# automl/TransformersCanDoBayesianInference

Hardware: AMD Instinct MI355X
Metric: synthetic datasets/sec (GP prior, bptt=2000) (higher is better)
Workload: dtype fp16; 1 GPU; priors.fast_gp, bptt=2000, num_features=18, emsize=512, nhead=4, nhid=1024, nlayers=6, 1000 bars (BASELINE.json configs[1]); per_gpu_batch=64, global_batch=64, aggregate_k_gradients=1, aggregate_streams=0, aggregate_stacked=False, seq_len=2000, parallelism=dp1, micro_batch_streams=2, eval_pos=weighted sampler(2000)

## Files before the change

transformerscandobayesianinference_amd/csrc/gemm.hip:

```cpp
#include <type_traits>
#include "pfn_device.h"
#include "pfn_kernels.h"

namespace pfn {

PFN_DEV int xcd_remap(int bid, int nwg) {
  const int q = nwg >> 3, r = nwg & 7, xcd = bid & 7;
  return (xcd < r ? xcd * (q + 1) : r * (q + 1) + (xcd - r) * q) + (bid >> 3);
}

constexpr int GEMM_BM = 128, GEMM_BN = 128, GEMM_RB = 128;

template <typename T>
__global__ __launch_bounds__(256, 2) void gemm_nt_kernel(GemmNT g) {
  operand_store_mode<T>();
  constexpr int BK = GEMM_RB / sizeof(T);
  extern __shared__ __attribute__((aligned(16))) char smem_raw[];
  LdsPtr smem = lds_cast(smem_raw);
  auto tileA = [&](int buf) { return smem + buf * 32768; };
  auto tileB = [&](int buf) { return smem + buf * 32768 + 16384; };

  const int tiles_n = (g.N + GEMM_BN - 1) / GEMM_BN;
  const int tiles_m = (g.M + GEMM_BM - 1) / GEMM_BM;
  const int tid_lin = xcd_remap(blockIdx.x, tiles_m * tiles_n);
  const int tm = tid_lin / tiles_n, tn = tid_lin % tiles_n;
  const int m0 = tm * GEMM_BM, n0 = tn * GEMM_BN;
  const int rowsA = min(GEMM_BM, g.M - m0), rowsB = min(GEMM_BN, g.N - n0);

  const T* A = reinterpret_cast<const T*>(g.A) + (long)m0 * g.lda;
  const T* B = reinterpret_cast<const T*>(g.B) + (long)n0 * g.ldb;

  const int wave = threadIdx.x >> 6, lane = threadIdx.x & 63;
  const int wm = wave >> 1, wn = wave & 1;

  f32x16 acc[2][2];
#pragma unroll
  for (int i = 0; i < 2; ++i)
#pragma unroll
    for (int j = 0; j < 2; ++j)
#pragma unroll
      for (int r = 0; r < 16; ++r) acc[i][j][r] = 0.f;

  TileStage<T, GEMM_BM, GEMM_RB, 256> sa, sb;
  const int nk = (g.K + BK - 1) / BK;
  sa.issue(A, g.lda, rowsA, g.K);
  sb.issue(B, g.ldb, rowsB, g.K);
  sa.template commit<false>(tileA(0));
  sb.template commit<false>(tileB(0));
  __syncthreads();

  for (int kt = 0; kt < nk; ++kt) {
    const int cur = kt & 1;
    if (kt + 1 < nk) {
      const int k1 = (kt + 1) * BK;
      sa.issue(A + k1, g.lda, rowsA, g.K - k1);
      sb.issue(B + k1, g.ldb, rowsB, g.K - k1);
    }
    const lds_char* ta = tileA(cur);
    const lds_char* tb = tileB(cur);
#pragma unroll
    for (int ks = 0; ks < BK; ks += 16) {
// ... 78 lines not shown
        const int n = ncol + e;
        if (flags & EPI_BIAS) x += bias[n];
        if ((flags & EPI_ROWSHIFT) && n >= g.rs_n0 && n < g.rs_n1) x -= g.rowshift[(m / g.rs_S) * g.rs_ld + (n - g.rs_n0)];
        if (flags & EPI_GELU_BWD) x *= (float)aux[m * g.ld_aux + n];
        if (flags & EPI_RESID) x += g.resid[m * g.ld_resid + n];
        if (flags & EPI_RESID_T) x += (float)aux[m * g.ld_aux + n];
        float second = x;
        if (flags & EPI_GELU) gelu_and_grad(x, x, second);
        if (flags & EPI_OUT2_T) out2_t[m * g.ld_out2 + n] = (T)second;
        if (flags & EPI_OUT_F32) { float* o = g.out_f32 + m * g.ld_out_f32 + n; *o = (flags & EPI_ACCUM) ? (*o + x) : x; }
        if (flags & EPI_OUT_T) out_t[m * g.ld_out_t + n] = (T)x;
      }
    }
  }
}


constexpr int BIG_BN = 256;
template <int NWM> struct BigEpi {
  static constexpr int EP_T = 32 * 144, EP_F = 32 * 272, EP_WAVE = (2 * EP_T > EP_F ? 2 * EP_T : EP_F), BYTES = NWM * 4 * EP_WAVE;
};
template <typename T, int FLAGS, int NWM>
PFN_DEV void nt_big_epilogue(const GemmNT& g, f32x16 (&acc)[4][2], int m0, int n0, int wave, int lane, LdsPtr ep_base, const lds_char* shift_lds = nullptr) {
  const int wm = wave >> 2, wn = wave & 3;
  const int h = lane >> 5, li = lane & 31;
  constexpr int flags = FLAGS;
  const T* aux = reinterpret_cast<const T*>(g.aux);
  T* out_t = reinterpret_cast<T*>(g.out_t);
  T* out2_t = reinterpret_cast<T*>(g.out2_t);
  constexpr bool HAS_AUX = (flags & (EPI_GELU_BWD | EPI_RESID_T | EPI_ROWDOT)) != 0;
  constexpr bool HAS_RES = (flags & EPI_RESID) != 0;
  float rowdot = 0.f;
  constexpr bool EARLY = NWM == 2;
  constexpr int NB = !EARLY ? 1 : HAS_RES ? 2 : 4;
  f32x4 bias_v[2][4];
  if ((flags & EPI_BIAS) && EARLY) {
#pragma unroll
    for (int j = 0; j < 2; ++j)
#pragma unroll
      for (int gq = 0; gq < 4; ++gq) bias_v[j][gq] = *reinterpret_cast<const f32x4*>(g.bias + min(n0 + wn * 64 + j * 32 + 8 * gq + 4 * h, g.N - 4));
  }
  constexpr int EP_T = 32 * 144, EP_F = 32 * 272, EP_WAVE = (2 * EP_T > EP_F ? 2 * EP_T : EP_F);
  static_assert(!(flags & EPI_ACCUM), "accumulating outputs take the generic kernel");
  LdsPtr ep = ep_base + wave * EP_WAVE;
  const bool lines = n0 + wn * 64 + 64 <= g.N && g.wide_t;
#pragma unroll
  for (int pass = 0; pass < 8 / NB; ++pass) {
    X4<T> aux_v[HAS_AUX ? NB : 1][4];
    f32x4 res_v[HAS_RES ? NB : 1][4];
#pragma unroll
    for (int bb = 0; bb < NB; ++bb) {
      const int blk = pass * NB + bb, i = blk >> 1, j = blk & 1;
      if (EARLY && (HAS_AUX || HAS_RES)) {
        const long m = min((long)m0 + wm * 128 + i * 32 + li, (long)g.M - 1);
#pragma unroll
        for (int gq = 0; gq < 4; ++gq) {
          const int n = min(n0 + wn * 64 + j * 32 + 8 * gq + 4 * h, g.N - 4);
          if constexpr (HAS_AUX) aux_v[bb][gq] = *reinterpret_cast<const X4<T>*>(aux + m * g.ld_aux + n);
          if constexpr (HAS_RES) res_v[bb][gq] = *reinterpret_cast<const f32x4*>(g.resid + m * g.ld_resid + n);
        }
      }
    }
#pragma unroll
    for (int bb = 0; bb < NB; ++bb) {
      const int blk = pass * NB + bb, i = blk >> 1, j = blk & 1;
      const long m_row = (long)m0 + wm * 128 + i * 32 + li;
      const bool mvalid = m_row < g.M;
      const long m = mvalid ? m_row : (long)g.M - 1;
      const int nb = n0 + wn * 64 + j * 32;
      float pre[16], post[16];
      f32x4 shift_v[4];
      const bool shifted = (flags & EPI_ROWSHIFT) && nb >= g.rs_n0 && nb < g.rs_n1;
      if (shifted) {
        if (shift_lds) {
          const int which = min((int)((unsigned)m / (unsigned)g.rs_S) - (int)((unsigned)m0 / (unsigned)g.rs_S), 1);
          const lds_char* sp = shift_lds + (which * BIG_BN + (nb - n0) + 4 * h) * 4;
#pragma unroll
          for (int gq = 0; gq < 4; ++gq) shift_v[gq] = __builtin_bit_cast(f32x4, lds_read16(sp + 32 * gq));
        } else {
          const float* sp = g.rowshift + (long)((unsigned)m / (unsigned)g.rs_S) * g.rs_ld + (nb - g.rs_n0) + 4 * h;
#pragma unroll
          for (int gq = 0; gq < 4; ++gq) shift_v[gq] = *reinterpret_cast<const f32x4*>(sp + 8 * gq);
        }
      }
#pragma unroll
      for (int gq = 0; gq < 4; ++gq) {
        const int n = min(nb + 8 * gq + 4 * h, g.N - 4);
        f32x4 v;
#pragma unroll
        for (int e = 0; e < 4; ++e) v[e] = acc[i][j][4 * gq + e];
        if constexpr (!EARLY) {
          if (flags & EPI_BIAS) bias_v[j][gq] = *reinterpret_cast<const f32x4*>(g.bias + n);
          if constexpr (HAS_AUX) aux_v[bb][gq] = *reinterpret_cast<const X4<T>*>(aux + m * g.ld_aux + n);
          if constexpr (HAS_RES) res_v[bb][gq] = *reinterpret_cast<const f32x4*>(g.resid + m * g.ld_resid + n);
        }
        if (flags & EPI_BIAS) v += bias_v[j][gq];
        if (shifted) v -= shift_v[gq];
        if (flags & EPI_GELU_BWD) {
#pragma unroll
          for (int e = 0; e < 4; ++e) v[e] *= (float)aux_v[HAS_AUX ? bb : 0][gq][e];
        }
        if (flags & EPI_RESID) v += res_v[HAS_RES ? bb : 0][gq];
        if (flags & EPI_RESID_T) {
#pragma unroll
          for (int e = 0; e < 4; ++e) v[e] += (float)aux_v[HAS_AUX ? bb : 0][gq][e];
        }
#pragma unroll
// ... 199 lines not shown

template <int NWN> struct LnEpi {
  static constexpr int STRIPS = 128 * NWN * 4 + 5 * NWN * 64 * 4;
  static constexpr int WAVE = 32 * 272 + 32 * 144;
  static constexpr int BYTES = STRIPS + NWN * WAVE;
};
template <typename T, int NWN, bool RESID_LN, int BK, bool Y16>
__global__ __launch_bounds__(NWN * 64) void gemm_nt_ln_kernel(GemmLN g) {
  operand_store_mode<T>();
  constexpr int BM = 128, RB = BK * 2, CPR = RB / 16, RPP = 1024 / RB, BN = NWN * 64;
  constexpr int PA = BM / RPP / NWN > 0 ? BM / RPP / NWN : 1, PB = BN / RPP / NWN;
  constexpr int TILE_A = BM * RB, STAGE = TILE_A + BN * RB;
  extern __shared__ __attribute__((aligned(16))) char smem_raw[];
  LdsPtr smem = lds_cast(smem_raw);
  const int m0 = blockIdx.x * BM;
  const int wave = __builtin_amdgcn_readfirstlane(threadIdx.x >> 6), lane = threadIdx.x & 63;
  const int h = lane >> 5, li = lane & 31;

  const T* pa[PA];
  const T* pb[PB];
  constexpr int APIECES = BM / RPP;
#pragma unroll
  for (int i = 0; i < PA; ++i) {
    const int piece = wave + NWN * i;
    const int row = piece * RPP + lane / CPR;
    const int chunk = swz16<RB>(row, lane % CPR);
    pa[i] = reinterpret_cast<const T*>(g.A) + (long)min(m0 + row, g.M - 1) * g.lda + chunk * 8;
  }
#pragma unroll
  for (int i = 0; i < PB; ++i) {
    const int row = (wave + NWN * i) * RPP + lane / CPR;
    const int chunk = swz16<RB>(row, lane % CPR);
    pb[i] = reinterpret_cast<const T*>(g.B) + (long)row * g.ldb + chunk * 8;
  }
  auto stage = [&](int buf, int k0) {
    LdsPtr ta = smem + buf * STAGE + wave * 1024;
    LdsPtr tb = smem + buf * STAGE + TILE_A + wave * 1024;
#pragma unroll
    for (int i = 0; i < PA; ++i)
      if (wave + NWN * i < APIECES) __builtin_amdgcn_global_load_lds((gvoid_t*)(pa[i] + k0), (lvoid_t*)(ta + i * NWN * 1024), 16, 0, 0);
#pragma unroll
    for (int i = 0; i < PB; ++i) __builtin_amdgcn_global_load_lds((gvoid_t*)(pb[i] + k0), (lvoid_t*)(tb + i * NWN * 1024), 16, 0, 0);
  };

  f32x16 acc[4][2];
#pragma unroll
  for (int i = 0; i < 4; ++i)
#pragma unroll
    for (int j = 0; j < 2; ++j)
#pragma unroll
      for (int r = 0; r < 16; ++r) acc[i][j][r] = 0.f;

  const int nk = g.K / BK;
  stage(0, 0);
  __syncthreads();
  for (int kt = 0; kt < nk; ++kt) {
    const int cur = kt & 1;
    if (kt + 1 < nk) stage(cur ^ 1, (kt + 1) * BK);
    const lds_char* ta = smem + cur * STAGE;
    const lds_char* tb = ta + TILE_A;
#pragma unroll
    for (int ks = 0; ks < BK; ks += 16) {
      Frag<T> fa[4], fb[2];
#pragma unroll
      for (int j = 0; j < 2; ++j) fb[j] = load_frag_row<T, RB>(tb, wave * 64 + j * 32 + li, ks);
#pragma unroll
      for (int i = 0; i < 4; ++i) fa[i] = load_frag_row<T, RB>(ta, i * 32 + li, ks);
#pragma unroll
      for (int i = 0; i < 4; ++i)
#pragma unroll
        for (int j = 0; j < 2; ++j) acc[i][j] = mma32(fb[j], fa[i], acc[i][j]);
    }
    __syncthreads();
  }

  float* red = reinterpret_cast<float*>(smem_raw);
  float* cvec = red + 128 * NWN;
  {
    const int n = threadIdx.x;
    float c0 = 0.f, c1 = 0.f;
    if constexpr (RESID_LN) { c0 = g.rgamma[n]; c1 = g.rbeta[n]; }
    const float c2 = g.bias[n], c3 = g.gamma[n], c4 = g.beta[n];
    cvec[n] = c0; cvec[BN + n] = c1; cvec[2 * BN + n] = c2; cvec[3 * BN + n] = c3; cvec[4 * BN + n] = c4;
  }
  typedef typename std::conditional<Y16 && RESID_LN, X4<T>, f32x4>::type RV;
  const float* rsrc = RESID_LN ? reinterpret_cast<const float*>(g.ry) : g.resid;
  float rm[2], rr[2];
  int mrow[4];
#pragma unroll
  for (int i = 0; i < 4; ++i) mrow[i] = min(m0 + i * 32 + li, g.M - 1);
  RV rv[2][8];
  auto fetch_rows = [&](int i, RV (&dst)[8]) {
    rm[i & 1] = 0.f; rr[i & 1] = 1.f;
    if constexpr (RESID_LN) { rm[i & 1] = g.rmean[mrow[i]]; rr[i & 1] = g.rrstd[mrow[i]]; }
#pragma unroll
    for (int j = 0; j < 2; ++j)
#pragma unroll
      for (int gq = 0; gq < 4; ++gq) {
        const long off = (long)mrow[i] * BN + wave * 64 + j * 32 + 8 * gq + 4 * h;
        if constexpr (Y16 && RESID_LN) dst[j * 4 + gq] = *reinterpret_cast<const X4<T>*>(reinterpret_cast<const T*>(g.ry) + off);
        else dst[j * 4 + gq] = *reinterpret_cast<const f32x4*>(rsrc + off);
      }
  };
  fetch_rows(0, rv[0]);
  __syncthreads();
  float mean[4], rstd[4];
  const float invN = 1.f / (float)BN;
#pragma unroll
  for (int i = 0; i < 4; ++i) {
    if (i + 1 < 4) fetch_rows(i + 1, rv[(i + 1) & 1]);
    float s = 0.f;
#pragma unroll
    for (int j = 0; j < 2; ++j)
#pragma unroll
      for (int gq = 0; gq < 4; ++gq) {
        const int n = wave * 64 + j * 32 + 8 * gq + 4 * h;
        f32x4 r;
#pragma unroll
        for (int e = 0; e < 4; ++e) r[e] = (float)rv[i & 1][j * 4 + gq][e];
        if constexpr (RESID_LN) {
          const f32x4 ga = *reinterpret_cast<const f32x4*>(cvec + n), be = *reinterpret_cast<const f32x4*>(cvec + BN + n);
#pragma unroll
          for (int e = 0; e < 4; ++e) r[e] = (r[e] - rm[i & 1]) * rr[i & 1] * ga[e] + be[e];
        }
        const f32x4 bi = *reinterpret_cast<const f32x4*>(cvec + 2 * BN + n);
#pragma unroll
        for (int e = 0; e < 4; ++e) {
          const float v = acc[i][j][4 * gq + e] + bi[e] + r[e];
          acc[i][j][4 * gq + e] = v;
          s += v;
        }
      }
    s += __shfl_xor(s, 32, 64);
    if (h == 0) red[(i * 32 + li) * NWN + wave] = s;
  }
  __syncthreads();
#pragma unroll
  for (int i = 0; i < 4; ++i) {
    float t = 0.f;
#pragma unroll
    for (int w = 0; w < NWN; ++w) t += red[(i * 32 + li) * NWN + w];
    mean[i] = t * invN;
  }
  __syncthreads();
#pragma unroll
  for (int i = 0; i < 4; ++i) {
    float s = 0.f;
#pragma unroll
    for (int j = 0; j < 2; ++j)
#pragma unroll
      for (int r = 0; r < 16; ++r) { const float d = acc[i][j][r] - mean[i]; s += d * d; }
    s += __shfl_xor(s, 32, 64);
    if (h == 0) red[(i * 32 + li) * NWN + wave] = s;
  }
  __syncthreads();
#pragma unroll
  for (int i = 0; i < 4; ++i) {
    float t = 0.f;
#pragma unroll
    for (int w = 0; w < NWN; ++w) t += red[(i * 32 + li) * NWN + w];
    rstd[i] = rsqrtf(t * invN + g.eps);
  }
  typedef __attribute__((address_space(3))) X4<T> lds_tx4;
  T* x_t = reinterpret_cast<T*>(g.x_t);
  LdsPtr sf = smem + LnEpi<NWN>::STRIPS + wave * LnEpi<NWN>::WAVE, st = sf + 32 * 272;
#pragma unroll
  for (int i = 0; i < 4; ++i) {
    const bool mvalid = m0 + i * 32 + li < g.M;
    const long m = mrow[i];
    if (mvalid && wave == 0 && h == 0) { g.mean[m] = mean[i]; g.rstd[m] = rstd[i]; }
#pragma unroll
    for (int j = 0; j < 2; ++j) {
      const int nb = wave * 64 + j * 32;
#pragma unroll
      for (int gq = 0; gq < 4; ++gq) {
        const int n = nb + 8 * gq + 4 * h;
        const f32x4 ga = *reinterpret_cast<const f32x4*>(cvec + 3 * BN + n), be = *reinterpret_cast<const f32x4*>(cvec + 4 * BN + n);
        f32x4 v, xo;
        X4<T> xt;
#pragma unroll
        for (int e = 0; e < 4; ++e) {
          v[e] = acc[i][j][4 * gq + e];
          xo[e] = (v[e] - mean[i]) * rstd[i] * ga[e] + be[e];
          xt[e] = (T)xo[e];
        }
        if constexpr (Y16) {
          X4<T> vt;
// ... 328 lines not shown
  for (int i = 0; i < 4; ++i)
#pragma unroll
    for (int j = 0; j < 2; ++j)
#pragma unroll
      for (int r = 0; r < 16; ++r) acc[i][j][r] = 0.f;

  const int nk = g.K / BK;
  stage(0, 0);
  __syncthreads();
  for (int kt = 0; kt < nk; ++kt) {
    const int cur = kt & 1;
    if (kt + 1 < nk) stage(cur ^ 1, (kt + 1) * BK);
    const lds_char* ta = smem + cur * STAGE;
    const lds_char* tb = ta + TILE_A;
#pragma unroll
    for (int ks = 0; ks < BK; ks += 16) {
      Frag<T> fa[4], fb[2];
#pragma unroll
      for (int j = 0; j < 2; ++j) fb[j] = load_frag_row<T, RB>(tb, wave * 64 + j * 32 + li, ks);
#pragma unroll
      for (int i = 0; i < 4; ++i) fa[i] = load_frag_row<T, RB>(ta, i * 32 + li, ks);
#pragma unroll
      for (int i = 0; i < 4; ++i)
#pragma unroll
        for (int j = 0; j < 2; ++j) acc[i][j] = mma32(fb[j], fa[i], acc[i][j]);
    }
    __syncthreads();
  }

  typedef __attribute__((address_space(3))) X4<T> lds_tx4;
  float* red1 = reinterpret_cast<float*>(smem_raw);
  float* red2 = red1 + 128 * NWN;
  float* gam = red2 + 128 * NWN;
  LdsPtr stash = smem + C::STASH + wave * 4 * C::STRIP;
  const T* aux = reinterpret_cast<const T*>(g.aux);
  T* dx_t = reinterpret_cast<T*>(g.dx_t);
  gam[threadIdx.x] = g.gamma[threadIdx.x];
  int mrow[4];
  bool mvalid[4];
  float mu[4], rs[4];
#pragma unroll
  for (int i = 0; i < 4; ++i) {
    const int m = m0 + i * 32 + li;
    mvalid[i] = m < g.M;
    mrow[i] = mvalid[i] ? m : g.M - 1;
    mu[i] = g.mean[mrow[i]]; rs[i] = g.rstd[mrow[i]];
  }
  typedef typename std::conditional<Y16, X4<T>, f32x4>::type YV;
  YV yv[2][4];
  X4<T> av[2][4];
  auto fetch_half = [&](int hb, YV (&dy)[4], X4<T> (&da)[4]) {
#pragma unroll
    for (int gq = 0; gq < 4; ++gq) {
      const long off = (long)mrow[hb >> 1] * BN + wave * 64 + (hb & 1) * 32 + 8 * gq + 4 * h;
      if constexpr (Y16) dy[gq] = *reinterpret_cast<const X4<T>*>(reinterpret_cast<const T*>(g.y) + off);
      else dy[gq] = *reinterpret_cast<const f32x4*>(reinterpret_cast<const float*>(g.y) + off);
      da[gq] = *reinterpret_cast<const X4<T>*>(aux + off);
    }
  };
  fetch_half(0, yv[0], av[0]);
  __syncthreads();
  const float invN = 1.f / (float)BN;
  float s1 = 0.f, s2 = 0.f;
#pragma unroll
  for (int hb = 0; hb < 8; ++hb) {
    const int i = hb >> 1, j = hb & 1;
    asm volatile("" ::: "memory");
    if (hb + 1 < 8) fetch_half(hb + 1, yv[(hb + 1) & 1], av[(hb + 1) & 1]);
    __builtin_amdgcn_sched_barrier(0);
#pragma unroll
    for (int gq = 0; gq < 4; ++gq) {
      const int n = wave * 64 + j * 32 + 8 * gq + 4 * h;
      const f32x4 ga = *reinterpret_cast<const f32x4*>(gam + n);
      X4<T> xh_t;
#pragma unroll
      for (int e = 0; e < 4; ++e) {
        const float v = mvalid[i] ? acc[i][j][4 * gq + e] + (float)av[hb & 1][gq][e] : 0.f;
        acc[i][j][4 * gq + e] = v;
        const float xh = ((float)yv[hb & 1][gq][e] - mu[i]) * rs[i];
        const float gv = ga[e] * v;
        s1 += gv;
        s2 += gv * xh;
        xh_t[e] = (T)xh;
      }
      *reinterpret_cast<lds_tx4*>(stash + i * C::STRIP + li * 144 + (j * 4 + gq) * 16 + h * 8) = xh_t;
    }
    if (j == 1) {
      s1 += __shfl_xor(s1, 32, 64);
      s2 += __shfl_xor(s2, 32, 64);
      if (h == 0) { red1[(i * 32 + li) * NWN + wave] = s1; red2[(i * 32 + li) * NWN + wave] = s2; }
      s1 = 0.f; s2 = 0.f;
    }
  }
  __syncthreads();
  float m1[4], m2[4];
#pragma unroll
  for (int i = 0; i < 4; ++i) {
    float t1 = 0.f, t2 = 0.f;
#pragma unroll
    for (int w = 0; w < NWN; ++w) { t1 += red1[(i * 32 + li) * NWN + w]; t2 += red2[(i * 32 + li) * NWN + w]; }
    m1[i] = t1 * invN; m2[i] = t2 * invN;
  }
  __syncthreads();
  float* csum = red1;
  const int ccol = wave * 64 + 4 * h, chalf = (li >> 4) * BN;
  {
#pragma unroll
// ... 338 lines not shown
    PFN_BIG_CASE(EPI_OUT_T | EPI_ROWDOT)
    PFN_BIG_CASE(EPI_OUT_F32)
    PFN_BIG_CASE(EPI_BIAS | EPI_OUT_F32)
#undef PFN_BIG_CASE
    default: return false;
  }
}

static void nt_prepare(GemmNT& g, int precision);
bool gemm_nt_rowdot_fused(const GemmNT& g_in, int precision) {
  GemmNT g = g_in;
  if (!prec_is16(precision) || g.M <= 0 || g.flags != (EPI_OUT_T | EPI_ROWDOT) || g.N % 64 || g.rd_D % 64 || g.N % g.rd_D) return false;
  if ((g.lda * 2) % 16 || (g.ldb * 2) % 16 || !aligned16(g.A) || !aligned16(g.B)) return false;
  nt_prepare(g, precision);
  return gemm_nt_pick(g) == 1 && g.wide_t;
}
int launch_gemm_nt(const GemmNT& g_in, int precision, hipStream_t stream) {
  GemmNT g = g_in;
  if (g.M <= 0 || g.N <= 0 || g.K <= 0) return PFN_OK;
  const size_t es = prec_esize(precision);
  if ((g.lda * es) % 16 || (g.ldb * es) % 16 || !aligned16(g.A) || !aligned16(g.B)) return PFN_ERR_ALIGNMENT;
  if ((g.flags & EPI_ROWSHIFT) && (!g.rowshift || g.rs_S <= 0 || g.rs_n0 % 64 || g.rs_n1 % 64 || g.rs_n0 < 0 || g.rs_n1 > g.N)) return PFN_ERR_ARGUMENT;
  nt_prepare(g, precision);
  if (prec_is16(precision)) {
    const int pick = gemm_nt_pick(g);
    if (pick && (precision == PFN_PREC_FP16 ? launch_big<f16>(g, pick == 2, stream) : launch_big<bf16>(g, pick == 2, stream)))
      return hipGetLastError() == hipSuccess ? PFN_OK : PFN_ERR_LAUNCH;
  }
  if (g.flags & EPI_ROWDOT) return PFN_ERR_UNSUPPORTED;
  const int tiles = ((g.M + GEMM_BM - 1) / GEMM_BM) * ((g.N + GEMM_BN - 1) / GEMM_BN);
  PFN_DISPATCH_OP(precision, hipLaunchKernelGGL(gemm_nt_kernel<T>, dim3(tiles), dim3(256), 65536, stream, g));
  return hipGetLastError() == hipSuccess ? PFN_OK : PFN_ERR_LAUNCH;
}
static void nt_prepare(GemmNT& g, int precision) {
  const size_t es = prec_esize(precision);
  bool vec = true;
  if ((g.flags & EPI_OUT_F32) && (g.ld_out_f32 % 4 || !aligned16(g.out_f32))) vec = false;
  if ((g.flags & EPI_OUT_T) && ((g.ld_out_t * es) % (4 * es) || !aligned16(g.out_t))) vec = false;
  if ((g.flags & EPI_OUT2_T) && ((g.ld_out2 * es) % (4 * es) || !aligned16(g.out2_t))) vec = false;
  if ((g.flags & EPI_RESID) && (g.ld_resid % 4 || !aligned16(g.resid))) vec = false;
  if ((g.flags & (EPI_GELU_BWD | EPI_RESID_T | EPI_ROWDOT)) && ((g.ld_aux * es) % (4 * es) || !aligned16(g.aux))) vec = false;
  if ((g.flags & EPI_BIAS) && !aligned16(g.bias)) vec = false;
  if ((g.flags & EPI_ROWSHIFT) && (!aligned16(g.rowshift) || g.rs_ld % 4 || g.rs_n0 % 4 || g.rs_n1 % 4)) vec = false;
  g.vec_ok = vec ? 1 : 0;
  g.wide_t = (!(g.flags & EPI_OUT_T) || g.ld_out_t % 8 == 0) && (!(g.flags & EPI_OUT2_T) || g.ld_out2 % 8 == 0) ? 1 : 0;
}

bool gemm_ln_supported(const GemmLN& g) {
  return (g.N == 128 || g.N == 256 || g.N == 512 || g.N == 1024) && g.K % 32 == 0 && g.K >= 32 && (g.lda * 2) % 16 == 0 && (g.ldb * 2) % 16 == 0 &&
         aligned16(g.A) && aligned16(g.B) && aligned16(g.bias) && aligned16(g.gamma) && aligned16(g.beta) && aligned16(g.y) && aligned16(g.x_t) &&
         (g.resid ? aligned16(g.resid) : (aligned16(g.ry) && aligned16(g.rgamma) && aligned16(g.rbeta)));
}
template <typename T, bool Y, int NWN, bool RL, int BK> static void launch_gemm_ln_t(const GemmLN& g, hipStream_t stream) {
  const size_t lds = std::max<size_t>(2 * (128 + NWN * 64) * (BK * 2), LnEpi<NWN>::BYTES);
  static LdsAllowance allowance;
  allowance.ensure(gemm_nt_ln_kernel<T, NWN, RL, BK, Y>, lds);
  hipLaunchKernelGGL((gemm_nt_ln_kernel<T, NWN, RL, BK, Y>), dim3((g.M + 127) / 128), dim3(NWN * 64), lds, stream, g);
}
static int g_ln_rows64 = 0;
void set_gemm_ln_rows64(int on) { g_ln_rows64 = on; }
template <typename T, bool Y, int NWN, bool RL, int BK, int MI, int NJ> static void launch_gemm_ln_wide_t(const GemmLN& g, hipStream_t stream) {
  constexpr int BM = MI * 32;
  const size_t lds = std::max<size_t>(2 * (BM + NWN * NJ * 32) * (BK * 2), LnEpiW<NWN, MI, NJ>::BYTES);
  static LdsAllowance allowance;
  allowance.ensure(gemm_nt_ln_wide_kernel<T, NWN, RL, BK, MI, NJ, Y>, lds);
  hipLaunchKernelGGL((gemm_nt_ln_wide_kernel<T, NWN, RL, BK, MI, NJ, Y>), dim3((g.M + BM - 1) / BM), dim3(NWN * 64), lds, stream, g);
}
template <typename T, bool Y> static int launch_gemm_ln_op(const GemmLN& g, hipStream_t stream) {
  const bool rl = g.resid == nullptr;
#define PFN_LN_CASE(NWN) \
  if (g.K % 64 == 0) { if (rl) launch_gemm_ln_t<T, Y, NWN, true, 64>(g, stream); else launch_gemm_ln_t<T, Y, NWN, false, 64>(g, stream); } \
  else { if (rl) launch_gemm_ln_t<T, Y, NWN, true, 32>(g, stream); else launch_gemm_ln_t<T, Y, NWN, false, 32>(g, stream); }
  if (g.N == 512 && g_ln_rows64) {
    if (rl) launch_gemm_ln_wide_t<T, Y, 4, true, 32, 2, 4>(g, stream); else launch_gemm_ln_wide_t<T, Y, 4, false, 32, 2, 4>(g, stream);
    return hipGetLastError() == hipSuccess ? PFN_OK : PFN_ERR_LAUNCH;
  }
  switch (g.N / 64) {
    case 2: PFN_LN_CASE(2) break;
    case 4: PFN_LN_CASE(4) break;
    case 8: PFN_LN_CASE(8) break;
    default:
      if (rl) launch_gemm_ln_wide_t<T, Y, 8, true, 32, 2, 4>(g, stream); else launch_gemm_ln_wide_t<T, Y, 8, false, 32, 2, 4>(g, stream);
      break;
  }
#undef PFN_LN_CASE
  return hipGetLastError() == hipSuccess ? PFN_OK : PFN_ERR_LAUNCH;
}
int launch_gemm_ln(const GemmLN& g, int precision, hipStream_t stream) {
  if (g.M <= 0) return PFN_OK;
  if (!prec_is16(precision) || !gemm_ln_supported(g)) return PFN_ERR_UNSUPPORTED;
  if (g.y16) return precision == PFN_PREC_FP16 ? launch_gemm_ln_op<f16, true>(g, stream) : PFN_ERR_UNSUPPORTED;
  return precision == PFN_PREC_FP16 ? launch_gemm_ln_op<f16, false>(g, stream) : launch_gemm_ln_op<bf16, false>(g, stream);
}

bool gemm_lnbwd_supported(const GemmLNB& g) {
  return (g.N == 128 || g.N == 256 || g.N == 512 || g.N == 1024) && g.K % 32 == 0 && g.K >= 32 && (g.lda * 2) % 16 == 0 && (g.ldb * 2) % 16 == 0 &&
         aligned16(g.A) && aligned16(g.B) && aligned16(g.aux) && aligned16(g.y) && aligned16(g.gamma) && aligned16(g.dx_t) && g.dgamma && g.dbeta;
}
template <typename T, bool Y, int NWN, int BK> static void launch_gemm_lnbwd_t(const GemmLNB& g, hipStream_t stream) {
  const size_t lds = LnbCfg<NWN, BK>::LDS;
  static LdsAllowance allowance;
  allowance.ensure(gemm_nt_lnbwd_kernel<T, NWN, BK, Y>, lds);
  hipLaunchKernelGGL((gemm_nt_lnbwd_kernel<T, NWN, BK, Y>), dim3((g.M + 127) / 128), dim3(NWN * 64), lds, stream, g);
}
template <typename T, bool Y, int NWN, int BK, int MI, int NJ> static void launch_gemm_lnbwd_wide_t(const GemmLNB& g, hipStream_t stream) {
  const size_t lds = LnbCfgW<NWN, BK, MI, NJ>::LDS;
  static LdsAllowance allowance;
// ... 27 lines not shown
```

transformerscandobayesianinference_amd/csrc/pfn_device.h:

```cpp
#pragma once
#include <hip/hip_runtime.h>
#include <stdint.h>

namespace pfn {

typedef __bf16 bf16;
typedef __attribute__((ext_vector_type(8))) __bf16 bf16x8;
typedef __attribute__((ext_vector_type(4))) __bf16 bf16x4;
typedef __attribute__((ext_vector_type(2))) __bf16 bf16x2;
typedef _Float16 f16;
typedef __attribute__((ext_vector_type(8))) _Float16 f16x8;
typedef __attribute__((ext_vector_type(4))) _Float16 f16x4;
typedef __attribute__((ext_vector_type(2))) _Float16 f16x2;
typedef __attribute__((ext_vector_type(16))) float f32x16;
typedef __attribute__((ext_vector_type(4))) float f32x4;
typedef __attribute__((ext_vector_type(2))) float f32x2;
typedef __attribute__((ext_vector_type(4))) unsigned int u32x4;
typedef __attribute__((ext_vector_type(2))) unsigned int u32x2;
template <typename T> struct OpVec;
template <> struct OpVec<bf16> { typedef bf16x8 x8; typedef bf16x4 x4; typedef bf16x2 x2; };
template <> struct OpVec<f16> { typedef f16x8 x8; typedef f16x4 x4; typedef f16x2 x2; };
template <> struct OpVec<float> { typedef f32x4 x8; typedef f32x4 x4; typedef f32x2 x2; };
template <typename T> using X8 = typename OpVec<T>::x8;
template <typename T> using X4 = typename OpVec<T>::x4;
// ... 213 lines not shown
}

typedef __amdgpu_buffer_rsrc_t BufRsrc;
PFN_DEV BufRsrc make_rsrc(const void* base, long bytes) {
  const int n = bytes > 0x7ffffff0L ? 0x7ffffff0 : (bytes < 0 ? 0 : (int)bytes);
  return __builtin_amdgcn_make_buffer_rsrc(const_cast<void*>(base), 0, n, 0x00020000);
}
PFN_DEV u32x4 buf_load16(BufRsrc r, int byte_offset) { return __builtin_amdgcn_raw_buffer_load_b128(r, byte_offset, 0, 0); }
constexpr int BUF_OOB = 0x7ffffff0;

struct DmaRsrc { u32x4 w; };
PFN_DEV DmaRsrc make_dma_rsrc(const void* base, long bytes) {
  const unsigned long long p = (unsigned long long)base;
  const int n = bytes > 0x7ffffff0L ? 0x7ffffff0 : (bytes < 0 ? 0 : (int)bytes);
  DmaRsrc r;
  r.w[0] = __builtin_amdgcn_readfirstlane((unsigned)p);
  r.w[1] = __builtin_amdgcn_readfirstlane((unsigned)(p >> 32) & 0xffffu);
  r.w[2] = __builtin_amdgcn_readfirstlane((unsigned)n);
  r.w[3] = 0x00020000u;
  return r;
}
PFN_DEV void dma_rsrc_advance(DmaRsrc& r, unsigned bytes) {
  const unsigned long long b = (((unsigned long long)r.w[1] << 32) | r.w[0]) + bytes;
  r.w[0] = (unsigned)b;
  r.w[1] = (unsigned)(b >> 32);
  r.w[2] = (unsigned)max((int)r.w[2] - (int)bytes, 0);
}
PFN_DEV void dma16(const DmaRsrc& r, LdsPtr lds_dst_uniform, int byte_offset) {
  unsigned keep;
  const unsigned dst = __builtin_amdgcn_readfirstlane((unsigned)(unsigned long long)lds_dst_uniform);
  const u32x4 w = {(unsigned)__builtin_amdgcn_readfirstlane(r.w[0]), (unsigned)__builtin_amdgcn_readfirstlane(r.w[1]),
                   (unsigned)__builtin_amdgcn_readfirstlane(r.w[2]), (unsigned)__builtin_amdgcn_readfirstlane(r.w[3])};
  asm volatile("s_mov_b32 %0, m0\n\ts_mov_b32 m0, %1\n\ts_nop 0\n\tbuffer_load_dwordx4 %2, %3, 0 offen lds\n\ts_mov_b32 m0, %0"
               : "=&s"(keep) : "s"(dst), "v"(byte_offset), "s"(w) : "memory");
}
PFN_DEV void dma4(const DmaRsrc& r, LdsPtr lds_dst_uniform, int byte_offset) {
  unsigned keep;
  const unsigned dst = __builtin_amdgcn_readfirstlane((unsigned)(unsigned long long)lds_dst_uniform);
  const u32x4 w = {(unsigned)__builtin_amdgcn_readfirstlane(r.w[0]), (unsigned)__builtin_amdgcn_readfirstlane(r.w[1]),
                   (unsigned)__builtin_amdgcn_readfirstlane(r.w[2]), (unsigned)__builtin_amdgcn_readfirstlane(r.w[3])};
  asm volatile("s_mov_b32 %0, m0\n\ts_mov_b32 m0, %1\n\ts_nop 0\n\tbuffer_load_dword %2, %3, 0 offen lds\n\ts_mov_b32 m0, %0"
               : "=&s"(keep) : "s"(dst), "v"(byte_offset), "s"(w) : "memory");
}
PFN_DEV void dma16_global(const void* src, LdsPtr lds_dst_uniform) {
  unsigned keep;
  const unsigned dst = __builtin_amdgcn_readfirstlane((unsigned)(unsigned long long)lds_dst_uniform);
  asm volatile("s_mov_b32 %0, m0\n\ts_mov_b32 m0, %1\n\ts_nop 0\n\tglobal_load_lds_dwordx4 %2, off\n\ts_mov_b32 m0, %0"
               : "=&s"(keep) : "s"(dst), "v"(src) : "memory");
}
template <int N> PFN_DEV void wait_vm_barrier() {
  __builtin_amdgcn_s_waitcnt(0x0070 | (N & 15) | ((N >> 4) << 14));
  asm volatile("s_waitcnt vmcnt(%0) lgkmcnt(0)\n\ts_barrier" :: "n"(N) : "memory");
}
PFN_DEV void dma_wait_all() {
  __builtin_amdgcn_s_waitcnt(0x0F70);
  asm volatile("s_waitcnt vmcnt(0)" ::: "memory");
}

template <typename T, int ROWS, int RB, int NT> struct TileStageBuf {
  static constexpr int NCH = RB / 16;
  static constexpr int TOTAL = ROWS * NCH;
  static constexpr int PER = (TOTAL + NT - 1) / NT;
  u32x4 regs[PER];
  int voff[PER];
  PFN_DEV void init(int ld_bytes) {
#pragma unroll
    for (int i = 0; i < PER; ++i) {
      const int id = threadIdx.x + i * NT;
      voff[i] = (TOTAL % NT == 0 || id < TOTAL) ? (id / NCH) * ld_bytes + (id % NCH) * 16 : BUF_OOB;
    }
  }
  PFN_DEV void issue(BufRsrc r, int tile_byte_offset) {
#pragma unroll
    for (int i = 0; i < PER; ++i) regs[i] = buf_load16(r, voff[i] + tile_byte_offset);
  }
  template <int STRIDE> PFN_DEV void commit_p(LdsPtr tile) const {
#pragma unroll
    for (int i = 0; i < PER; ++i) {
      const int id = threadIdx.x + i * NT;
      if (TOTAL % NT != 0 && id >= TOTAL) break;
      lds_write16(tile + (id / NCH) * STRIDE + (id % NCH) * 16, regs[i]);
    }
  }
};

template <typename T, int ROWS, int RB, int NT> struct TileStage {
  static constexpr int NCH = RB / 16;
  static constexpr int TOTAL = ROWS * NCH;
  static constexpr int PER = (TOTAL + NT - 1) / NT;
  static constexpr int EPC = 16 / sizeof(T);
  u32x4 regs[PER];

  PFN_DEV void issue(const T* src, long ld, int rows_valid, int cols_valid) {
#pragma unroll
    for (int i = 0; i < PER; ++i) {
      const int id = threadIdx.x + i * NT;
      const int row = id / NCH, c = id % NCH;
      u32x4 v = {0u, 0u, 0u, 0u};
      if ((TOTAL % NT == 0 || id < TOTAL) && row < rows_valid && (c + 1) * EPC <= cols_valid)
        v = *reinterpret_cast<const u32x4*>(src + (long)row * ld + c * EPC);
      else if ((TOTAL % NT == 0 || id < TOTAL) && row < rows_valid && c * EPC < cols_valid) {
        T tmp[EPC];
#pragma unroll
        for (int e = 0; e < EPC; ++e) tmp[e] = (c * EPC + e < cols_valid) ? src[(long)row * ld + c * EPC + e] : (T)0.f;
        v = *reinterpret_cast<u32x4*>(tmp);
      }
// ... 107 lines not shown
```

Measured before the change: 2612 datasets/s.

## Stream LN-epilogue residual rows into LDS via async DMA overlapping last k-step

In the fused GEMM+LayerNorm kernel, the residual/ry rows used by the epilogue are now fetched with global_load_lds DMA into swizzled LDS images instead of register loads. The first row blocks are issued before the last k-tile multiply so their latency overlaps the final MMAs, with vmcnt waits staged per row block. Per-column constants are held in registers and written to LDS after the loop, and the LDS size is raised to fit the row images. An optional PFN_EPI_ROWS_L2 macro that redirects source rows to the first tile is added for experimentation but is off by default. This frees registers and hides epilogue load latency, at the cost of more LDS (possibly lower occupancy) and extra wait/barrier complexity.

```diff
diff --git a/transformerscandobayesianinference_amd/csrc/epi_rows_map.h b/transformerscandobayesianinference_amd/csrc/epi_rows_map.h
--- /dev/null
+++ b/transformerscandobayesianinference_amd/csrc/epi_rows_map.h
@@ -0,0 +1,37 @@
+#pragma once
+
+namespace pfn {
+
+template <int ES> struct EpiRows {
+  static_assert(ES == 2 || ES == 4, "operand precision or f32 rows");
+  static constexpr int ROWB = 64 * ES;
+  static constexpr int CPR = ROWB / 16;
+  static constexpr int RPP = 1024 / ROWB;
+  static constexpr int PIECES = 32 / RPP;
+  static constexpr int BLOCK = 32 * ROWB;
+  static constexpr int swz(int row, int chunk) { return ES == 2 ? chunk ^ ((row >> 1) & 7) : chunk ^ (row & 15); }
+  static constexpr int off(int row, int chunk) { return row * ROWB + swz(row, chunk) * 16; }
+  static constexpr int dma_dst(int piece, int lane) { return piece * 1024 + lane * 16; }
+  static constexpr int dma_row(int piece, int lane) { return piece * RPP + lane / CPR; }
+  static constexpr int dma_chunk(int piece, int lane) { return swz(dma_row(piece, lane), lane % CPR); }
+  static constexpr int read_chunk(int j, int gq, int h) { return ES == 2 ? j * 4 + gq : j * 8 + gq * 2 + h; }
+};
+
+template <int NWN> struct EpiRowsLn {
+  static constexpr int HALF = 8192, REGION = NWN * HALF;
+  static constexpr int HEAD = (128 * NWN * 4 + 5 * NWN * 64 * 4 + 1023) / 1024 * 1024;
+  static constexpr int stage(int bk) { return (128 + NWN * 64) * bk * 2; }
+  static constexpr bool under(int bk) { return HEAD + REGION <= stage(bk) && REGION <= stage(bk); }
+  static constexpr int lo() { return HEAD; }
+  static constexpr int hi(int bk) { return under(bk) ? stage(bk) : HEAD + REGION; }
+  static constexpr int end(int bk) { return hi(bk) + REGION; }
+  static constexpr int early_region(int bk, int last) { return under(bk) ? last ^ 1 : 0; }
+  template <int ES> static constexpr int half_of(int block) { return ES == 2 ? block >> 1 : block & 1; }
+  template <int ES> static constexpr int off_in_half(int block) { return ES == 2 ? (block & 1) * EpiRows<2>::BLOCK : 0; }
+  template <int ES> static constexpr int image(int bk, int last, int wave, int block) {
+    const int region = half_of<ES>(block) == 0 ? early_region(bk, last) : early_region(bk, last) ^ 1;
+    return (region ? hi(bk) : lo()) + wave * HALF + off_in_half<ES>(block);
+  }
+};
+
+}
diff --git a/transformerscandobayesianinference_amd/csrc/gemm.hip b/transformerscandobayesianinference_amd/csrc/gemm.hip
--- a/transformerscandobayesianinference_amd/csrc/gemm.hip
+++ b/transformerscandobayesianinference_amd/csrc/gemm.hip
@@ -1,12 +1,21 @@
 #include <type_traits>
 #include "pfn_device.h"
 #include "pfn_kernels.h"
+#include "epi_rows_map.h"
 
 namespace pfn {
 
 PFN_DEV int xcd_remap(int bid, int nwg) {
   const int q = nwg >> 3, r = nwg & 7, xcd = bid & 7;
   return (xcd < r ? xcd * (q + 1) : r * (q + 1) + (xcd - r) * q) + (bid >> 3);
+}
+
+PFN_DEV int epi_src_row(int row, int row_in_tile) {
+#ifdef PFN_EPI_ROWS_L2
+  return row_in_tile & 127;
+#else
+  return row;
+#endif
 }
 
 constexpr int GEMM_BM = 128, GEMM_BN = 128, GEMM_RB = 128;
@@ -191,7 +200,7 @@
     for (int bb = 0; bb < NB; ++bb) {
       const int blk = pass * NB + bb, i = blk >> 1, j = blk & 1;
       if (EARLY && (HAS_AUX || HAS_RES)) {
-        const long m = min((long)m0 + wm * 128 + i * 32 + li, (long)g.M - 1);
+        const long m = epi_src_row((int)min((long)m0 + wm * 128 + i * 32 + li, (long)g.M - 1), i * 32 + li);
 #pragma unroll
         for (int gq = 0; gq < 4; ++gq) {
           const int n = min(n0 + wn * 64 + j * 32 + 8 * gq + 4 * h, g.N - 4);
@@ -497,11 +506,7 @@
       for (int r = 0; r < 16; ++r) acc[i][j][r] = 0.f;
 
   const int nk = g.K / BK;
-  stage(0, 0);
-  __syncthreads();
-  for (int kt = 0; kt < nk; ++kt) {
-    const int cur = kt & 1;
-    if (kt + 1 < nk) stage(cur ^ 1, (kt + 1) * BK);
+  auto multiply = [&](int cur) {
     const lds_char* ta = smem + cur * STAGE;
     const lds_char* tb = ta + TILE_A;
 #pragma unroll
@@ -516,57 +521,90 @@
 #pragma unroll
         for (int j = 0; j < 2; ++j) acc[i][j] = mma32(fb[j], fa[i], acc[i][j]);
     }
+  };
+  stage(0, 0);
+  __syncthreads();
+  for (int kt = 0; kt + 1 < nk; ++kt) {
+    const int cur = kt & 1;
+    stage(cur ^ 1, (kt + 1) * BK);
+    multiply(cur);
     __syncthreads();
   }
 
+  typedef typename std::conditional<Y16 && RESID_LN, X4<T>, f32x4>::type RV;
+  constexpr int ES = sizeof(RV) / 4;
+  using R = EpiRows<ES>;
+  using P = EpiRowsLn<NWN>;
+  constexpr bool UNDER = P::under(BK);
+  static_assert(P::HEAD >= LnEpi<NWN>::STRIPS && (!UNDER || (P::lo() + P::REGION <= STAGE && P::hi(BK) >= STAGE)) && P::end(BK) <= 160 * 1024, "row images");
+  const int last = (nk - 1) & 1;
+  const int early = P::early_region(BK, last);
+  LdsPtr img_half[2] = {smem + (early ? P::hi(BK) : P::lo()) + wave * P::HALF, smem + (early ? P::lo() : P::hi(BK)) + wave * P::HALF};
+  auto image = [&](int i) -> LdsPtr { return img_half[P::template half_of<ES>(i)] + P::template off_in_half<ES>(i); };
+  const char* rsrc = (RESID_LN ? reinterpret_cast<const char*>(g.ry) : reinterpret_cast<const char*>(g.resid)) + wave * R::ROWB;
+  auto request_rows = [&](int i) {
+    LdsPtr dst = image(i);
+#pragma unroll
+    for (int p = 0; p < R::PIECES; ++p) {
+      const int r = i * 32 + R::dma_row(p, lane);
+      const int m = epi_src_row(min(m0 + r, g.M - 1), r);
+      dma16_global(rsrc + (long)m * (BN * ES) + R::dma_chunk(p, lane) * 16, dst + p * 1024);
+    }
+  };
+  int mrow[4];
+  float rm[4], rr[4];
+  float cv[5] = {0.f, 0.f, 0.f, 0.f, 0.f};
+#pragma unroll
+  for (int i = 0; i < 4; ++i) {
+    mrow[i] = min(m0 + i * 32 + li, g.M - 1);
+    rm[i] = 0.f; rr[i] = 1.f;
+    if constexpr (RESID_LN) { rm[i] = g.rmean[mrow[i]]; rr[i] = g.rrstd[mrow[i]]; }
+  }
+  if constexpr (RESID_LN) { cv[0] = g.rgamma[threadIdx.x]; cv[1] = g.rbeta[threadIdx.x]; }
+  cv[2] = g.bias[threadIdx.x]; cv[3] = g.gamma[threadIdx.x]; cv[4] = g.beta[threadIdx.x];
+  if constexpr (UNDER) {
+    request_rows(0);
+    if constexpr (ES == 2) request_rows(1);
+  }
+  multiply(last);
+  dma_wait<0>();
+  __syncthreads();
   float* red = reinterpret_cast<float*>(smem_raw);
   float* cvec = red + 128 * NWN;
-  {
-    const int n = threadIdx.x;
-    float c0 = 0.f, c1 = 0.f;
-    if constexpr (RESID_LN) { c0 = g.rgamma[n]; c1 = g.rbeta[n]; }
-    const float c2 = g.bias[n], c3 = g.gamma[n], c4 = g.beta[n];
-    cvec[n] = c0; cvec[BN + n] = c1; cvec[2 * BN + n] = c2; cvec[3 * BN + n] = c3; cvec[4 * BN + n] = c4;
-  }
-  typedef typename std::conditional<Y16 && RESID_LN, X4<T>, f32x4>::type RV;
-  const float* rsrc = RESID_LN ? reinterpret_cast<const float*>(g.ry) : g.resid;
-  float rm[2], rr[2];
-  int mrow[4];
-#pragma unroll
-  for (int i = 0; i < 4; ++i) mrow[i] = min(m0 + i * 32 + li, g.M - 1);
-  RV rv[2][8];
-  auto fetch_rows = [&](int i, RV (&dst)[8]) {
-    rm[i & 1] = 0.f; rr[i & 1] = 1.f;
-    if constexpr (RESID_LN) { rm[i & 1] = g.rmean[mrow[i]]; rr[i & 1] = g.rrstd[mrow[i]]; }
-#pragma unroll
-    for (int j = 0; j < 2; ++j)
-#pragma unroll
-      for (int gq = 0; gq < 4; ++gq) {
-        const long off = (long)mrow[i] * BN + wave * 64 + j * 32 + 8 * gq + 4 * h;
-        if constexpr (Y16 && RESID_LN) dst[j * 4 + gq] = *reinterpret_cast<const X4<T>*>(reinterpret_cast<const T*>(g.ry) + off);
-        else dst[j * 4 + gq] = *reinterpret_cast<const f32x4*>(rsrc + off);
-      }
-  };
-  fetch_rows(0, rv[0]);
+#pragma unroll
+  for (int c = 0; c < 5; ++c) cvec[c * BN + threadIdx.x] = cv[c];
+  if constexpr (!UNDER) {
+    request_rows(0);
+    if constexpr (ES == 2) request_rows(1);
+  }
+  if constexpr (ES == 2) { request_rows(2); request_rows(3); }
+  else request_rows(1);
+  if constexpr (!UNDER) dma_wait<8>();
   __syncthreads();
   float mean[4], rstd[4];
   const float invN = 1.f / (float)BN;
 #pragma unroll
   for (int i = 0; i < 4; ++i) {
-    if (i + 1 < 4) fetch_rows(i + 1, rv[(i + 1) & 1]);
+    if constexpr (ES == 2) { if (i == 2) dma_wait<0>(); }
+    else { if (i == 1 || i == 2) dma_wait<8>(); else if (i == 3) dma_wait<0>(); }
+    const lds_char* img = image(i);
     float s = 0.f;
 #pragma unroll
     for (int j = 0; j < 2; ++j)
 #pragma unroll
       for (int gq = 0; gq < 4; ++gq) {
         const int n = wave * 64 + j * 32 + 8 * gq + 4 * h;
+        const u32x4 q = lds_read16(img + R::off(li, R::read_chunk(j, gq, h)));
+        RV rv;
+        if constexpr (ES == 2) { const u32x2 half = {h ? q[2] : q[0], h ? q[3] : q[1]}; rv = __builtin_bit_cast(RV, half); }
+        else rv = __builtin_bit_cast(RV, q);
         f32x4 r;
 #pragma unroll
-        for (int e = 0; e < 4; ++e) r[e] = (float)rv[i & 1][j * 4 + gq][e];
+        for (int e = 0; e < 4; ++e) r[e] = (float)rv[e];
         if constexpr (RESID_LN) {
           const f32x4 ga = *reinterpret_cast<const f32x4*>(cvec + n), be = *reinterpret_cast<const f32x4*>(cvec + BN + n);
 #pragma unroll
-          for (int e = 0; e < 4; ++e) r[e] = (r[e] - rm[i & 1]) * rr[i & 1] * ga[e] + be[e];
+          for (int e = 0; e < 4; ++e) r[e] = (r[e] - rm[i]) * rr[i] * ga[e] + be[e];
         }
         const f32x4 bi = *reinterpret_cast<const f32x4*>(cvec + 2 * BN + n);
 #pragma unroll
@@ -578,6 +616,12 @@
       }
     s += __shfl_xor(s, 32, 64);
     if (h == 0) red[(i * 32 + li) * NWN + wave] = s;
+    if constexpr (ES == 4) {
+      if (i < 2) {
+        lds_reads_done();
+        request_rows(i + 2);
+      }
+    }
   }
   __syncthreads();
 #pragma unroll
@@ -1012,7 +1056,7 @@
   auto fetch_half = [&](int hb, YV (&dy)[4], X4<T> (&da)[4]) {
 #pragma unroll
     for (int gq = 0; gq < 4; ++gq) {
-      const long off = (long)mrow[hb >> 1] * BN + wave * 64 + (hb & 1) * 32 + 8 * gq + 4 * h;
+      const long off = (long)epi_src_row(mrow[hb >> 1], (hb >> 1) * 32 + li) * BN + wave * 64 + (hb & 1) * 32 + 8 * gq + 4 * h;
       if constexpr (Y16) dy[gq] = *reinterpret_cast<const X4<T>*>(reinterpret_cast<const T*>(g.y) + off);
       else dy[gq] = *reinterpret_cast<const f32x4*>(reinterpret_cast<const float*>(g.y) + off);
       da[gq] = *reinterpret_cast<const X4<T>*>(aux + off);
@@ -1457,7 +1501,7 @@
          (g.resid ? aligned16(g.resid) : (aligned16(g.ry) && aligned16(g.rgamma) && aligned16(g.rbeta)));
 }
 template <typename T, bool Y, int NWN, bool RL, int BK> static void launch_gemm_ln_t(const GemmLN& g, hipStream_t stream) {
-  const size_t lds = std::max<size_t>(2 * (128 + NWN * 64) * (BK * 2), LnEpi<NWN>::BYTES);
+  const size_t lds = std::max<size_t>({2 * (128 + NWN * 64) * (BK * 2), LnEpi<NWN>::BYTES, EpiRowsLn<NWN>::end(BK)});
   static LdsAllowance allowance;
   allowance.ensure(gemm_nt_ln_kernel<T, NWN, RL, BK, Y>, lds);
   hipLaunchKernelGGL((gemm_nt_ln_kernel<T, NWN, RL, BK, Y>), dim3((g.M + 127) / 128), dim3(NWN * 64), lds, stream, g);
diff --git a/transformerscandobayesianinference_amd/csrc/pfn_device.h b/transformerscandobayesianinference_amd/csrc/pfn_device.h
--- a/transformerscandobayesianinference_amd/csrc/pfn_device.h
+++ b/transformerscandobayesianinference_amd/csrc/pfn_device.h
@@ -289,6 +289,8 @@
   __builtin_amdgcn_s_waitcnt(0x0070 | (N & 15) | ((N >> 4) << 14));
   asm volatile("s_waitcnt vmcnt(%0) lgkmcnt(0)\n\ts_barrier" :: "n"(N) : "memory");
 }
+template <int N> PFN_DEV void dma_wait() { asm volatile("s_waitcnt vmcnt(%0)" :: "n"(N) : "memory"); }
+PFN_DEV void lds_reads_done() { asm volatile("s_waitcnt lgkmcnt(0)" ::: "memory"); }
 PFN_DEV void dma_wait_all() {
   __builtin_amdgcn_s_waitcnt(0x0F70);
   asm volatile("s_waitcnt vmcnt(0)" ::: "memory");
```

Result: no change. 2611 datasets/s (median of 2 runs) (-0.0%).
